# Fedomn/sqlrs

Hardware: AMD Instinct MI355X
Metric: Mrows/sec for filter->hash-join->group-by pipeline; achieved HBM GB/s vs peak (higher is better)
Workload: dtype int64 keys / f64 sum; 1 GPU; C5 filter(val>0.5) -> hash-join(fact x dim on int64 key) -> group-by(key) COUNT,SUM(f64); fact_rows=1000000000, dim_rows=10000000, groups=10000000, parallelism=single GPU

## Files before the change

sqlrs_amd/csrc/agg_partition.hip:

```cpp
#include <algorithm>
#include <cstdlib>
#include <cstring>

#include "agg_partition.hpp"
#include "device_utils.hpp"
#include "radix_part.hpp"

namespace sq {

#ifndef PART_WG_N
#define PART_WG_N 512
#endif
constexpr int PART_WG = PART_WG_N;
#ifndef DENSE_WG_N
#define DENSE_WG_N 1024
#endif
constexpr int DENSE_WG = DENSE_WG_N;
#ifndef HOT_MIN_PEERS_N
#define HOT_MIN_PEERS_N 8
#endif
constexpr int HOT_MIN_PEERS = HOT_MIN_PEERS_N;
constexpr uint64_t LDS_EMPTY = ~0ull;

__device__ __forceinline__ uint32_t bucket_of(uint64_t h, uint32_t P) {
// ... 799 lines not shown
      const int64_t st = in.nzstart[col + k];
      if (st <= lo) before++;
      else if (st < hi) {
        inside++;
        atomicOr(&gmask[(st - lo) >> 6], 1ull << ((st - lo) & 63));
      }
    }
    before = wave_sum_u32(before);
    inside = wave_sum_u32(inside);
    if (lane_id() == 0 && before) atomicAdd(&s_before, before);
    if (lane_id() == 0 && inside) atomicAdd(&s_inside, inside);
  }
  __syncthreads();
  const uint32_t k_first = s_before - 1u, k_count = s_inside + 1u;
  const bool bt_lds = !BLK && k_count <= SLIM_BT_CAP;
  const bool seg_mode = NACC == 2 && ((C0 == AK_COUNT && C1 == AK_SUM_F64) || (C0 == AK_SUM_F64 && C1 == AK_COUNT)) &&
                        hi - lo >= 4096 && (int64_t)k_count * 2048 <= hi - lo && !prm.seg_off && !BLK;
  if (bt_lds)
    for (uint32_t k = threadIdx.x; k < k_count; k += DENSE_WG) gbt[k] = in.nzbt[col + min(k_first + k, nruns - 1)];
  if (!BLK) {
    constexpr uint32_t GPT = 8;
    uint32_t carry = s_before - 1u;
    for (uint32_t g0 = 0; g0 < ngroups; g0 += DENSE_WG * GPT) {
      const uint32_t gb = g0 + threadIdx.x * GPT;
      uint32_t pc[GPT], sum = 0;
#pragma unroll
      for (uint32_t i = 0; i < GPT; i++) {
        pc[i] = gb + i < ngroups ? (uint32_t)__popcll(gmask[gb + i]) : 0u;
        sum += pc[i];
      }
      const uint32_t inc = wave_iscan_u32(sum);
      if (lane_id() == 63) s_wsum[wave_id()] = inc;
      __syncthreads();
      uint32_t wbase = 0, tot = 0;
      for (int w = 0; w < DENSE_WG / 64; w++) {
        if (w < wave_id()) wbase += s_wsum[w];
        tot += s_wsum[w];
      }
      uint32_t run = carry + wbase + inc - sum;
#pragma unroll
      for (uint32_t i = 0; i < GPT; i++) {
        if (gb + i < ngroups) gpre[gb + i] = run;
        run += pc[i];
      }
      carry += tot;
      __syncthreads();
    }
  }
#ifndef SLIM_WAVE_SPAN
#define SLIM_WAVE_SPAN 1
#endif
  constexpr int64_t SLIM_USTEP = SLIM_WAVE_SPAN ? 64 : DENSE_WG;
  const int64_t slim_toff = SLIM_WAVE_SPAN ? (int64_t)wave_id() * (LDS_U * 64) + lane_id() : (int64_t)threadIdx.x;
  auto load = [&](int64_t i0, SlimAggRows &r) {
#pragma unroll
    for (int u = 0; u < LDS_U; u++) {
      const int64_t i = min(i0 + (int64_t)u * SLIM_USTEP, hi - 1);
      slim_load_nt(in.rows, i, r.w[u], r.v[u]);
      if (BLK) {
        r.bt[u] = in.blk_bt[i >> in.log_b];
        continue;
      }
      const uint32_t g = (uint32_t)((i - lo) >> 6);
      const uint32_t k = gpre[g] + (uint32_t)__popcll(gmask[g] & le_mask);
#if defined(SLIM_DBG) && (SLIM_DBG & 16)
      r.bt[u] = k;
#else
      r.bt[u] = bt_lds ? gbt[min(k - k_first, k_count - 1)] : in.nzbt[col + min(k, nruns - 1)];
#endif
    }
  };
  uint32_t hc_slot = 0xffffffffu, hc_min = 0xffffffffu;
  uint64_t hc_acc[PART_MAX_ACC];
  auto hot_flush = [&]() {
    if (hc_slot == 0xffffffffu) return;
    if (lane_id() == 0) {
      atomicMin(&tfirst[hc_slot], hc_min);
#pragma unroll
      for (int a = 0; a < PART_MAX_ACC; a++) {
        if (a >= n_acc) break;
        unsigned long long *cell = tacc + (size_t)a * R + hc_slot;
        switch (code_of(a) & 7) {
        case AK_COUNT:
        case AK_SUM_I64: atomicAdd(cell, (unsigned long long)hc_acc[a]); break;
        case AK_SUM_F64: unsafeAtomicAdd((double *)cell, __longlong_as_double((long long)hc_acc[a])); break;
        case AK_MIN_I64:
        case AK_MIN_F64: atomicMin(cell, (unsigned long long)hc_acc[a]); break;
        default: atomicMax(cell, (unsigned long long)hc_acc[a]);
        }
      }
    }
    hc_slot = 0xffffffffu;
  };
  auto hot_take = [&](uint32_t s0, uint32_t idmin) {
    if (hc_slot != s0) {
      hot_flush();
      hc_slot = s0;
      hc_min = 0xffffffffu;
#pragma unroll
      for (int a = 0; a < PART_MAX_ACC; a++) {
        if (a >= n_acc) break;
        hc_acc[a] = acc_identity_cell(code_of(a) & 7);
      }
    }
    hc_min = idmin < hc_min ? idmin : hc_min;
  };
  auto hot_add = [&](int a, int kind, uint64_t red) {
    switch (kind) {
    case AK_COUNT:
    case AK_SUM_I64: hc_acc[a] += red; break;
    case AK_SUM_F64: hc_acc[a] = (uint64_t)__double_as_longlong(__longlong_as_double((long long)hc_acc[a]) + __longlong_as_double((long long)red)); break;
    case AK_MIN_I64:
    case AK_MIN_F64: hc_acc[a] = red < hc_acc[a] ? red : hc_acc[a]; break;
    default: hc_acc[a] = red > hc_acc[a] ? red : hc_acc[a];
    }
  };
  SlimAggRows cur, nxt;
  if (lo < hi) load(lo + slim_toff, cur);
  __builtin_amdgcn_s_waitcnt(0x0F70);
  for (int64_t base = lo; base < hi; base += (int64_t)LDS_U * DENSE_WG) {
    const int64_t i0 = base + slim_toff;
    load(i0 + (int64_t)LDS_U * DENSE_WG, nxt);
    uint32_t sl[LDS_U], id[LDS_U], tf[LDS_U];
#pragma unroll
    for (int u = 0; u < LDS_U; u++) {
      const uint32_t w = cur.w[u];
      sl[u] = w & mask;
      id[u] = (cur.bt[u] + (w >> (rbits + 13))) * in.tile + ((w >> rbits) & lmask);
      tf[u] = tfirst[sl[u]];
    }
    constexpr bool SEG_CAPABLE = NACC == 2 && ((C0 == AK_COUNT && C1 == AK_SUM_F64) || (C0 == AK_SUM_F64 && C1 == AK_COUNT));
    const int lane = (int)lane_id();
    auto seg_rows = [&](bool act, uint32_t sl_u, uint64_t v_u, uint32_t id_u, uint32_t tf_u) {
      const uint32_t key = act ? sl_u : (0x80000000u | (uint32_t)lane);
      const uint32_t prevk = (uint32_t)__builtin_amdgcn_update_dpp(0, (int)key, 0x138, 0xf, 0xf, false);
      const uint64_t bm = __ballot(lane == 0 || key != prevk);
      const int headl = 63 - __builtin_clzll(bm & le_mask);
      double incl = act ? __longlong_as_double((long long)v_u) : 0.0;
      uint32_t idh = act ? id_u : 0xffffffffu;
      wave_seg_iscan_f64_min_u32(incl, idh, headl, lane);
      const bool tail = act && (lane == 63 || ((bm >> (lane + 1)) & 1ull));
      if (tail) {
        const uint32_t s = sl_u;
        if (idh < tf_u) atomicMin(&tfirst[s], idh);
        atomicAdd(tacc + (size_t)(C0 == AK_COUNT ? 0 : 1) * R + s, (unsigned long long)(lane - headl + 1));
        unsafeAtomicAdd((double *)(tacc + (size_t)(C0 == AK_COUNT ? 1 : 0) * R + s), incl);
      }
    };
    if (seg_mode) {
#pragma unroll
      for (int u = 0; u < LDS_U; u++) {
        const bool act = i0 + (int64_t)u * SLIM_USTEP < hi;
        {
          const uint32_t s0 = (uint32_t)__builtin_amdgcn_readfirstlane((int)sl[u]);
          if (__ballot(act && sl[u] == s0) == ~0ull) {
            hot_take(s0, wave_min_u32_dpp(id[u]));
            hot_add(C0 == AK_COUNT ? 0 : 1, AK_COUNT, 64ull);
            hot_add(C0 == AK_COUNT ? 1 : 0, AK_SUM_F64, (uint64_t)__double_as_longlong(wave_sum_f64_dpp(__longlong_as_double((long long)cur.v[u]))));
            continue;
          }
        }
        seg_rows(act, sl[u], cur.v[u], id[u], tf[u]);
      }
      cur = nxt;
      continue;
    }
#pragma unroll
    for (int u = 0; u < LDS_U; u++) {
      const uint32_t s = sl[u];
      bool act = i0 + (int64_t)u * SLIM_USTEP < hi;
      if (BLK) act = act && cur.w[u] != 0xffffffffu;
#ifdef SLIM_DBG
      uint64_t actm = (SLIM_DBG & 1) ? 0ull : __ballot(act);
#else
      uint64_t actm = __ballot(act);
#endif
      for (int it = 0; it < 3 && actm; it++) {
        const int first = __builtin_ctzll(actm);
        const uint32_t s0 = (uint32_t)__builtin_amdgcn_readlane((int)s, first);
        const bool hot = act && s == s0;
        const uint64_t peers = __ballot(hot);
        if (__popcll(peers) < HOT_MIN_PEERS) break;
// ... 596 lines not shown
```

sqlrs_amd/csrc/radix_part.hip:

```cpp
#include <cstdio>
#include <cstdlib>

#include "device_utils.hpp"
#include "radix_part.hpp"
#include "radix_part_kernels.hpp"

namespace sq {

namespace {

struct Level {
  std::vector<int64_t> seg_mat, seg_start;
  std::vector<uint32_t> seg_tiles, seg_tile_base;
  int64_t mat_entries = 0;
  uint32_t num_tiles = 0, nseg = 0;
  std::vector<uint8_t> blob;
  BufP dev, tiles;
  const int64_t *d_seg_start = nullptr, *d_seg_mat = nullptr;
  const uint32_t *d_seg_tiles = nullptr, *d_seg_tile_base = nullptr;
};

Level plan_level(const std::vector<int64_t> &seg_start, uint32_t digits, int RP_TILE) {
  Level L;
  L.seg_start = seg_start;
// ... 191 lines not shown
  auto run_level = [&](int level, uint32_t digits, const std::vector<int64_t> &seg_start, const RpIn &rin,
                       const RpOut &rout, BufP *offs_out, Level *L) {
    *L = plan_level(seg_start, digits, RP_TILE);
    L->tiles = ctx->alloc(sizeof(Tile) * (size_t)std::max<uint32_t>(L->num_tiles, 1));
    upload_level(ctx, *L);
    rp_make_tiles_kernel<<<dim3((unsigned)L->seg_tiles.size()), dim3(256), 0, ctx->stream>>>(
        L->d_seg_start, L->d_seg_mat, L->d_seg_tiles, L->d_seg_tile_base, RP_TILE, (Tile *)L->tiles->p);
    SQ_HIP(hipGetLastError());
    exec_level(level, digits, *L, rin, rout, n, offs_out);
  };

  auto bucket_starts = [&](const Level &L, const BufP &offs, uint32_t digits, int64_t rows,
                           std::vector<uint32_t> *host) -> BufP {
    uint32_t nseg = L.nseg;
    int64_t total = (int64_t)nseg * digits + 1;
    BufP bs = ctx->alloc(4 * (size_t)total);
    rp_bucket_starts_kernel<<<dim3((unsigned)ceil_div(total, 256)), dim3(256), 0, ctx->stream>>>(
        offs->as<uint32_t>(), L.d_seg_mat, L.d_seg_tiles, L.d_seg_start, digits, nseg, rows, bs->as<uint32_t>());
    SQ_HIP(hipGetLastError());
    if (4 * (size_t)total <= ctx->pinned_bytes) {
      const uint32_t *h = (const uint32_t *)ctx->fetch(bs->p, 4 * (size_t)total);
      host->assign(h, h + total);
      return bs;
    }
    host->resize((size_t)total);
    SQ_HIP(hipMemcpyAsync(host->data(), bs->p, 4 * (size_t)total, hipMemcpyDeviceToHost, ctx->stream));
    ctx->sync();
    return bs;
  };

  struct EarlyStarts {
    BufP bs;
    int64_t total = 0;
    std::function<void(const BufP &)> queue;
  };
  auto early_starts_for = [&](const Level &L, uint32_t digits, int64_t rows, EarlyStarts &es) {
    es.total = (int64_t)L.nseg * digits + 1;
    const char *es_e = hook("SQLRS_RP_EARLY_STARTS");
    const bool off = es_e && es_e[0] == '0';
    es.queue = [&L, &es, digits, rows, off, ctx](const BufP &offs) {
      if (off) return;
      BufP bs = ctx->alloc(4 * (size_t)es.total);
      rp_bucket_starts_kernel<<<dim3((unsigned)ceil_div(es.total, 256)), dim3(256), 0, ctx->stream>>>(
          offs->as<uint32_t>(), L.d_seg_mat, L.d_seg_tiles, L.d_seg_start, digits, L.nseg, rows, bs->as<uint32_t>());
      SQ_HIP(hipGetLastError());
      if (ctx->fetch_early(bs->p, 4 * (size_t)es.total)) es.bs = bs;
    };
  };
  auto finish_starts = [&](EarlyStarts &es, const Level &L, const BufP &offs, uint32_t digits, int64_t rows, std::vector<uint32_t> *host) -> BufP {
    if (!es.bs) return bucket_starts(L, offs, digits, rows, host);
    const uint32_t *h = (const uint32_t *)ctx->fetch_early_wait();
    host->assign(h, h + es.total);
    return es.bs;
  };

  const char *claim_e = hook("SQLRS_RP_CLAIM");
  const int claim_env = claim_e ? std::atoi(claim_e) : -1;
  const bool claimable = p2_bits == 0 && pack && kp.dense && nv <= 1 && P <= (uint32_t)WG && P >= 2 &&
                         claim_env != 0 && (claim_env == 1 || n >= (1ll << 22));
  if (claimable) {
    const uint32_t tiles1c = (uint32_t)ceil_div(n, RP_TILE);
    uint32_t wgs = std::min<uint32_t>(tiles1c, (uint32_t)ctx->num_cus);
    if (const char *wg_e = hook("SQLRS_RP_CHUNK_WGS"))
      wgs = std::max(1u, std::min<uint32_t>(wgs, (uint32_t)std::atoi(wg_e)));
    const uint32_t tpw = (uint32_t)ceil_div(tiles1c, std::max(wgs, 1u));
    wgs = (uint32_t)ceil_div(tiles1c, std::max(tpw, 1u));
    uint32_t B = 16;
    while (B < 256 && (uint64_t)(2 * B) * 16 * wgs * P <= (uint64_t)n) B *= 2;
    const uint32_t slack = 4096 + wgs * B;
    const uint64_t slots_max = (uint64_t)n + (uint64_t)n / 8 + (uint64_t)P * ((uint64_t)slack + B) + 64;
    const uint64_t pool_rows = slots_max + (uint64_t)1024 * wgs;
    if (pool_rows <= 0xffffffffull) {
      BufP est = ctx->alloc_zero(4 * ((size_t)P + 1));
      const size_t plan_words = 3 * (size_t)P + (P & 1), plan_bytes = 4 * plan_words + 16;
      BufP plan = ctx->alloc(plan_bytes);
      SQ_HIP(hipMemsetAsync(plan->as<uint8_t>() + 4 * plan_words, 0, 16, ctx->stream));
      uint32_t *rstart = plan->as<uint32_t>(), *rend = rstart + P, *cursor = rend + P;
      uint64_t *cst = (uint64_t *)(plan->as<uint32_t>() + plan_words);
      {
        ProfScope ps(ctx, "rp_sample_hist");
        uint32_t sdiv = 8;
        while (sdiv < 32 && (int64_t)P * 4096 * (2 * sdiv) <= n) sdiv *= 2;
        const int64_t samples = (int64_t)tiles1c * (RP_TILE / sdiv);
        const unsigned sblocks = (unsigned)std::max<int64_t>(1, std::min<int64_t>(ceil_div(samples, 256 * 4 * 2), 4 * (int64_t)ctx->num_cus));
        rp_sample_hist_kernel<<<dim3(sblocks), dim3(256), 0, ctx->stream>>>(in.keys, in.filter, n, (uint32_t)RP_TILE, tiles1c, P, kp, sdiv,
                                                                           est->as<uint32_t>());
        rp_region_plan_kernel<<<dim3(1), dim3(512), 0, ctx->stream>>>(est->as<uint32_t>(), P, n, slack, B, rstart, rend, cursor);
        SQ_HIP(hipGetLastError());
      }
      const char *cslim_e = hook("SQLRS_RP_SLIM");
      const bool claim_slim = nv == 1 && kp.rbits + SLIM_LOCAL_BITS + 7 <= 32 && !(cslim_e && std::atoi(cslim_e) == 0);
      Cols cc;
      PartitionedRows::Slim csl;
      if (claim_slim) {
        uint32_t log_b = 0;
        while ((1u << log_b) < B) log_b++;
        csl.buf0 = ctx->alloc(8 * (size_t)pool_rows);
        csl.buf1 = ctx->alloc(4 * (size_t)pool_rows);
        csl.rows.v = csl.buf0->as<uint64_t>();
        csl.rows.w = csl.buf1->as<uint32_t>();
        csl.blk_bt = ctx->alloc(4 * (size_t)((slots_max >> log_b) + 2));
        csl.log_b = log_b;
        csl.tile = (uint32_t)RP_TILE;
        csl.on = true;
      } else if (use_rec) cc.rec = ctx->alloc(16 * (size_t)pool_rows);
      else {
// ... 115 lines not shown
        v.v = b0->as<uint64_t>();
        v.w = b1->as<uint32_t>();
        return v;
      };
      BufP cb0, cb1;
      BufP clen = ctx->alloc_zero(4 * (size_t)max_chunks);
      BufP cdig = ctx->alloc(4 * (size_t)max_chunks), cbase = ctx->alloc(4 * (size_t)max_chunks);
      BufP cstart = ctx->alloc(2 * (size_t)max_chunks * SLIM_RUNS);
      SQ_HIP(hipMemsetAsync(cstart->p, 0xff, 2 * (size_t)max_chunks * SLIM_RUNS, ctx->stream));
      BufP ctr = ctx->alloc_zero(8);
      BufP chist = ctx->alloc(4 * (size_t)max_chunks * digits2);
      SlimChunkOut so;
      so.rows = slim_alloc(pool_rows, cb0, cb1);
      so.chunk_len = clen->as<uint32_t>();
      so.chunk_dig = cdig->as<uint32_t>();
      so.chunk_base = cbase->as<uint32_t>();
      so.cstart = cstart->as<uint16_t>();
      so.counter = ctr->as<unsigned int>();
      so.max_chunks = (uint32_t)max_chunks;
      so.cap = (uint32_t)CAP;
      so.arena = (uint32_t)arena;
      so.hist = chist->as<uint32_t>();
      so.kshift = kp.rbits + p2_bits;
      so.max_delta = slim_delta;
      {
        const char *cc_e = hook("SQLRS_RP_CONC");
        so.conc_eighths = cc_e ? (uint32_t)std::max(1, std::min(std::atoi(cc_e), 9)) : 3u;
      }
      const int psrc = !in.filter.col ? -1 : ((const void *)in.filter.col == in.vals[0] ? 1 : 3);
      const size_t clds = (size_t)RP_TILE * 14 + (size_t)WG * (4 + 4 + 8 + 8 + 4 + 4) + (size_t)P * 4;
      {
        ProfScope ps(ctx, in.filter.col ? "rp_chunk_scatter_filter" : "rp_chunk_scatter");
        const int64_t sink = (int64_t)max_chunks * (CAP + RP_CHUNK_SKEW);
        const size_t clds768 = (size_t)RP_TILE * 14 + (size_t)768 * (4 + 4 + 8 + 8 + 4 + 4) + (size_t)P * 4;
#define SQ_SL(W, R, PS, LDS)                                                                                        \
  do {                                                                                                              \
    auto kfn = rp_chunk_scatter_slim_kernel<W, R, PS>;                                                              \
    allow_big_lds(ctx, kfn);                                                                                        \
    kfn<<<dim3(cwgs), dim3(W), LDS, ctx->stream>>>(in.keys, (const uint64_t *)in.vals[0], in.filter, n, so, P, p2_bits, d1, \
                                                   tiles1, ctpw, sink, kp);                                         \
  } while (0)
        if (psrc < 0) SQ_SL(768, 8, -1, clds768); else if (psrc == 1) SQ_SL(768, 8, 1, clds768); else SQ_SL(512, 12, 3, clds);
#undef SQ_SL
        SQ_HIP(hipGetLastError());
      }
      Level L2;
      L2.nseg = d1;
      const LevelLayout lay(d1);
      L2.dev = ctx->alloc(lay.total);
      bind_level(L2, lay);
      L2.tiles = ctx->alloc(sizeof(Tile) * (size_t)max_chunks);
      BufP totals = ctx->alloc(24);
      BufP tile_chunk = ctx->alloc(4 * (size_t)max_chunks);
      BufP plan = ctx->alloc(sizeof(ChunkPlan));
      SQ_HIP(hipMemsetAsync(plan->p, 0, sizeof(ChunkPlan), ctx->stream));
      const unsigned pblocks = (unsigned)std::min<uint64_t>(ceil_div((int64_t)max_chunks, 256 * 8), 128);
      rp_chunk_count_kernel<<<dim3(pblocks), dim3(256), 0, ctx->stream>>>(so.chunk_len, so.chunk_dig, so.counter, so.max_chunks,
                                                                        so.max_chunks, (uint32_t)RP_TILE, plan->as<ChunkPlan>());
      rp_chunk_prefix_kernel<<<dim3(1), dim3(64), 0, ctx->stream>>>(
          plan->as<ChunkPlan>(), so.counter, d1, digits2, (int64_t *)L2.d_seg_start, (int64_t *)L2.d_seg_mat,
          (uint32_t *)L2.d_seg_tiles, (uint32_t *)L2.d_seg_tile_base, totals->as<uint64_t>());
      rp_chunk_assign_kernel<<<dim3(pblocks), dim3(256), 0, ctx->stream>>>(
          so.chunk_len, so.chunk_dig, so.counter, so.max_chunks, so.max_chunks, digits2, (uint32_t)CAP, (uint32_t)RP_TILE,
          L2.d_seg_tiles, L2.d_seg_tile_base, plan->as<ChunkPlan>(), (Tile *)L2.tiles->p, tile_chunk->as<uint32_t>());
      SQ_HIP(hipGetLastError());
      const uint64_t *ht = (const uint64_t *)ctx->fetch(totals->p, 24);
      const uint64_t ntiles = ht[0], kept = ht[1], overflow = ht[2];
      if (overflow) return false;
      L2.num_tiles = (uint32_t)ntiles;
      L2.mat_entries = (int64_t)ntiles * digits2;
      out->n = (int64_t)kept;
      out->P = P;
      if (kept == 0) {
        out->bstart_host.assign((size_t)P + 1, 0u);
        out->bstart = nullptr;
        return true;
      }
      const size_t np = (size_t)kept + 1024;
      PartitionedRows::Slim &sl = out->slim;
      sl = PartitionedRows::Slim();
      sl.rows = slim_alloc(np, sl.buf0, sl.buf1);
      SlimLaunch sln;
      sln.in.rows = so.rows;
      sln.in.tile_chunk = tile_chunk->as<uint32_t>();
      sln.in.cstart = so.cstart;
      sln.out.rows = sl.rows;
      sln.kshift = so.kshift;
      sln.rbits = kp.rbits;
      BufP offs2;
      BufP premat = ctx->alloc(4 * (size_t)L2.mat_entries);
      rp_hist_from_chunks_kernel<<<dim3((unsigned)ceil_div(L2.mat_entries, 256)), dim3(256), 0, ctx->stream>>>(
          so.hist, tile_chunk->as<uint32_t>(), L2.mat_entries, digits2, premat->as<uint32_t>());
      SQ_HIP(hipGetLastError());
      EarlyStarts es;
      early_starts_for(L2, digits2, (int64_t)kept, es);
      exec_level(2, digits2, L2, RpIn(), RpOut(), (int64_t)kept, &offs2, premat, &sln, &es.queue);
      sl.nzstart = ctx->alloc(4 * (size_t)L2.mat_entries);
      sl.nzbt = ctx->alloc(4 * (size_t)L2.mat_entries);
      sl.nzcount = ctx->alloc(4 * (size_t)P);
      sl.bcol = ctx->alloc(4 * (size_t)P);
      ProfScope ps_runs(ctx, "rp_slim_runs");
      rp_slim_runs_kernel<<<dim3(P), dim3(256), 0, ctx->stream>>>(
          offs2->as<uint32_t>(), L2.mat_entries, sln.total->as<uint64_t>(), L2.d_seg_mat, L2.d_seg_tiles, L2.d_seg_tile_base,
          tile_chunk->as<uint32_t>(), so.chunk_base, digits2, sl.nzstart->as<uint32_t>(), sl.nzbt->as<uint32_t>(),
          sl.nzcount->as<uint32_t>(), sl.bcol->as<uint32_t>());
      SQ_HIP(hipGetLastError());
      if (hook("SQLRS_RP_TRACE"))
        std::fprintf(stderr, "[rp_slim] keys %p vals %p chunks %p %p rows %p %p kept %llu tiles %u\n", (const void *)in.keys, in.vals[0],
                     cb0 ? cb0->p : nullptr, cb1 ? cb1->p : nullptr, sl.buf0 ? sl.buf0->p : nullptr, sl.buf1 ? sl.buf1->p : nullptr,
                     (unsigned long long)kept, L2.num_tiles);
      sl.tile = (uint32_t)RP_TILE;
      sl.on = true;
      out->key = out->v0 = out->v1 = out->idx = out->flags = out->rec = nullptr;
      out->bstart = finish_starts(es, L2, offs2, digits2, (int64_t)kept, &out->bstart_host);
      return true;
    }
    if (chunked) {
// ... 29 lines not shown
        const uint64_t *k = in.keys, *a0 = (const uint64_t *)in.vals[0], *a1 = (const uint64_t *)in.vals[1];
        const int64_t sink = (int64_t)max_chunks * (CAP + RP_CHUNK_SKEW);
#define SQ_CS1(NV, R, PK, PS)                                                                                       \
  do {                                                                                                              \
    auto kfn = rp_chunk_scatter_kernel<NV, 512, R, PK, PS>;                                                         \
    if (NV == 1 && PK && h2) kfn = rp_chunk_scatter_kernel<NV, 512, R, PK, PS, (NV == 1 && PK)>;                    \
    allow_big_lds(ctx, kfn);                                                                                        \
    kfn<<<dim3(cwgs), dim3(512), clds, ctx->stream>>>(k, a0, a1, in.filter, n, co, P, p2_bits, d1, tiles1, ctpw,   \
                                                      sink, kp);                                                    \
  } while (0)
#define SQ_CS(NV, R, PK)                                                                                            \
  do {                                                                                                              \
    if (psrc < 0) SQ_CS1(NV, R, PK, -1);                                                                            \
    else if (psrc == 1 && NV >= 1) SQ_CS1(NV, R, PK, (NV >= 1 ? 1 : 3));                                            \
    else SQ_CS1(NV, R, PK, 3);                                                                                      \
  } while (0)
        if (nv == 2) SQ_CS(2, 8, false);
        else if (nv == 0) { if (pack) SQ_CS(0, 12, true); else SQ_CS(0, 12, false); }
        else if (!pack && h2) {
#define SQ_CH(PS)                                                                                                   \
  do {                                                                                                              \
    auto kfn = rp_chunk_scatter_kernel<1, 512, 12, false, PS, true>;                                                \
    allow_big_lds(ctx, kfn, 159 * 1024);                                                                            \
    kfn<<<dim3(cwgs), dim3(512), clds, ctx->stream>>>(k, a0, a1, in.filter, n, co, P, p2_bits, d1, tiles1, ctpw, sink, kp); \
  } while (0)
          if (psrc < 0) SQ_CH(-1); else SQ_CH(1);
#undef SQ_CH
        }
        else if (!pack && psrc != 3) {
          const size_t clds768 = (size_t)RP_TILE * (8 * (1 + nv) + 4 + 2) + (size_t)768 * (4 + 4 + 8 + 8) + (clds - ((size_t)RP_TILE * (8 * (1 + nv) + 4 + 2) + (size_t)WG * (4 + 4 + 8 + 8)));
#define SQ_CG(PS)                                                                                                   \
  do {                                                                                                              \
    auto kfn = rp_chunk_scatter_kernel<1, 768, 8, false, PS>;                                                       \
    allow_big_lds(ctx, kfn);                                                                                        \
    kfn<<<dim3(cwgs), dim3(768), clds768, ctx->stream>>>(k, a0, a1, in.filter, n, co, P, p2_bits, d1, tiles1, ctpw, sink, kp); \
  } while (0)
          if (psrc < 0) SQ_CG(-1); else if (psrc == 1) SQ_CG(1); else SQ_CG(3);
#undef SQ_CG
        }
        else if (pack) SQ_CS(1, 12, true); else SQ_CS1(1, 12, false, 3);
#undef SQ_CS
#undef SQ_CS1
        SQ_HIP(hipGetLastError());
      }
      const uint32_t digits2 = 1u << p2_bits;
      Level L2;
      L2.nseg = d1;
      const LevelLayout lay(d1);
      L2.dev = ctx->alloc(lay.total);
      bind_level(L2, lay);
      L2.tiles = ctx->alloc(sizeof(Tile) * (size_t)max_chunks);
      BufP totals = ctx->alloc(24);
      BufP tile_chunk = h2 ? ctx->alloc(4 * (size_t)max_chunks) : nullptr;
      BufP plan = ctx->alloc(sizeof(ChunkPlan));
      SQ_HIP(hipMemsetAsync(plan->p, 0, sizeof(ChunkPlan), ctx->stream));
      const unsigned pblocks = (unsigned)std::min<uint64_t>(ceil_div((int64_t)max_chunks, 256 * 8), 128);
      rp_chunk_count_kernel<<<dim3(pblocks), dim3(256), 0, ctx->stream>>>(co.chunk_len, co.chunk_dig, co.counter, co.base_chunks,
                                                                        co.max_chunks, (uint32_t)RP_TILE, plan->as<ChunkPlan>());
      rp_chunk_prefix_kernel<<<dim3(1), dim3(64), 0, ctx->stream>>>(
          plan->as<ChunkPlan>(), co.counter, d1, digits2, (int64_t *)L2.d_seg_start, (int64_t *)L2.d_seg_mat,
          (uint32_t *)L2.d_seg_tiles, (uint32_t *)L2.d_seg_tile_base, totals->as<uint64_t>());
      rp_chunk_assign_kernel<<<dim3(pblocks), dim3(256), 0, ctx->stream>>>(
          co.chunk_len, co.chunk_dig, co.counter, co.base_chunks, co.max_chunks, digits2, (uint32_t)CAP, (uint32_t)RP_TILE,
          L2.d_seg_tiles, L2.d_seg_tile_base, plan->as<ChunkPlan>(), (Tile *)L2.tiles->p,
          tile_chunk ? tile_chunk->as<uint32_t>() : nullptr);
      SQ_HIP(hipGetLastError());
      const uint64_t *ht = (const uint64_t *)ctx->fetch(totals->p, 24);
      const uint64_t ntiles = ht[0], kept = ht[1], overflow = ht[2];
      if (overflow) return false;
      L2.num_tiles = (uint32_t)ntiles;
      L2.mat_entries = (int64_t)ntiles * digits2;
      out->n = (int64_t)kept;
      out->P = P;
      RpIn rin2;
      rin2.key = ck->as<uint64_t>();
      rin2.v0 = co.v0;
      rin2.v1 = co.v1;
      rin2.idx = co.idx;
      rin2.flags = nullptr;
      rin2.key_validity = rin2.v0_validity = rin2.v1_validity = nullptr;
      Cols c2;
      RpOut rout2;
      alloc_cols((int64_t)kept, true, c2, rout2);
      BufP offs2, premat;
      if (h2 && L2.mat_entries) {
        premat = ctx->alloc(4 * (size_t)L2.mat_entries);
        rp_hist_from_chunks_kernel<<<dim3((unsigned)ceil_div(L2.mat_entries, 256)), dim3(256), 0, ctx->stream>>>(
            co.hist, tile_chunk->as<uint32_t>(), L2.mat_entries, digits2, premat->as<uint32_t>());
        SQ_HIP(hipGetLastError());
      }
      EarlyStarts es;
      early_starts_for(L2, digits2, (int64_t)kept, es);
      exec_level(2, digits2, L2, rin2, rout2, (int64_t)kept, &offs2, premat, nullptr, &es.queue);
      publish(c2);
      out->bstart = finish_starts(es, L2, offs2, digits2, (int64_t)kept, &out->bstart_host);
      return true;
    }
  }

  Cols c1;
  RpOut rout;
  alloc_cols(n, p2_bits == 0, c1, rout);
  RpIn rin;
  rin.key = in.keys;
  rin.v0 = (const uint64_t *)in.vals[0];
  rin.v1 = (const uint64_t *)in.vals[1];
  rin.idx = nullptr;
  rin.flags = nullptr;
  rin.key_validity = in.key_validity;
  rin.v0_validity = in.val_validity[0];
  rin.v1_validity = in.val_validity[1];
  BufP offs1;
  Level L1;
  run_level(1, d1, {0, n}, rin, rout, &offs1, &L1);
  std::vector<uint32_t> hs;
  BufP bs1 = bucket_starts(L1, offs1, d1, n, &hs);
  out->n = n;
  out->P = P;
// ... 27 lines not shown
```

sqlrs_amd/csrc/radix_part_kernels.hpp:

```cpp
#pragma once
#include "device_utils.hpp"
#include "radix_part.hpp"

#ifdef RP_NT_STORES
#define RP_ST(ptr, val) __builtin_nontemporal_store((val), (ptr))
#else
#define RP_ST(ptr, val) (*(ptr) = (val))
#endif

namespace sq {


constexpr int vmcnt_imm(int n) { return (n & 0xF) | ((n >> 4) << 14) | 0x0F70; }

struct Tile {
  int64_t start;
  uint32_t len;
  uint32_t stride;
  int64_t mat;
};

__device__ __forceinline__ uint32_t xcd_tile(uint32_t b, uint32_t nb) {
  uint32_t q = nb >> 3, r = nb & 7, x = b & 7, i = b >> 3;
  return x * q + min(x, r) + i;
// ... 1335 lines not shown
    const uint32_t d = min((uint32_t)sdig[p], (uint32_t)(RP_WG - 1));
    int64_t g = (p < split[d] ? gb0[d] : gb1[d]) + p;
    if (p >= len || g < 0) g = sink + (int64_t)blockIdx.x * RP_WG + threadIdx.x;
    slim_store(out.rows, g, sw[p], sv0[p]);
  };

  if (t0 < t1) {
    uint32_t len = tile_len(t0);
    cur_tile = t0;
    rp_chunk_load<1, RP_WG, RP_ROWS, PSRC>(key, v0, nullptr, flt.col, tile_start(t0), len, nxt);
    __builtin_amdgcn_s_waitcnt(0x0F70);
    take_rows(len, t0, true, cur);
    cnt[threadIdx.x] = 0;
    __syncthreads();
#pragma unroll
    for (int j = 0; j < RP_ROWS; j++) rank_row(j);
    __syncthreads();
    scan_and_stage();
    uint32_t staged_len = s_total;
    uint32_t tcur = min(t0 + 1, t1 - 1);
    len = tile_len(tcur);
    cur_tile = tcur;
    rp_chunk_load<1, RP_WG, RP_ROWS, PSRC>(key, v0, nullptr, flt.col, tile_start(tcur), len, nxt);
    __builtin_amdgcn_s_waitcnt(0x0F70);
    take_rows(len, tcur, tcur != t0, cur);
    for (uint32_t ti = t0 + 1; ti < t1; ti++) {
      const uint32_t tnext = min(ti + 1, t1 - 1);
      const uint32_t nlen = tile_len(tnext);
      rp_chunk_load<1, RP_WG, RP_ROWS, PSRC>(key, v0, nullptr, flt.col, tile_start(tnext), nlen, nxt);
      cnt[threadIdx.x] = 0;
      __syncthreads();
#pragma unroll
      for (int j = 0; j < RP_ROWS; j++) {
        if ((uint32_t)(j * RP_WG) < staged_len) store_row(j, staged_len);
        rank_row(j);
      }
      __builtin_amdgcn_s_waitcnt(0x0F70);
      __syncthreads();
      scan_and_stage();
      staged_len = s_total;
      take_rows(nlen, tnext, tnext != ti, cur);
      cur_tile = tnext;
    }
#pragma unroll
    for (int j = 0; j < RP_ROWS; j++)
      if ((uint32_t)(j * RP_WG) < staged_len) store_row(j, staged_len);
  }
  if (owner && !dead) fill_sentinels(pos, room);
  if (threadIdx.x == 0 && kept) atomicAdd(out.kept, kept);
}

struct ChunkPlan {
  uint32_t seg_tiles[512];
  uint32_t cursor[512];
  unsigned long long seg_rows[512];
};
__global__ __launch_bounds__(256) void rp_chunk_count_kernel(const uint32_t *__restrict__ chunk_len,
                                                             const uint32_t *__restrict__ chunk_dig,
                                                             const unsigned int *__restrict__ counter, uint32_t base_chunks,
                                                             uint32_t max_chunks, uint32_t tile, ChunkPlan *plan) {
  __shared__ uint32_t s_tiles[512];
  __shared__ unsigned long long s_rows[512];
  for (uint32_t i = threadIdx.x; i < 512; i += 256) {
    s_tiles[i] = 0;
    s_rows[i] = 0;
  }
  __syncthreads();
  const uint32_t nchunks = min(base_chunks + counter[0], max_chunks);
  for (uint32_t c = blockIdx.x * 256 + threadIdx.x; c < nchunks; c += gridDim.x * 256) {
    const uint32_t len = chunk_len[c];
    if (!len) continue;
    atomicAdd(&s_tiles[chunk_dig[c]], (len + tile - 1) / tile);
    atomicAdd(&s_rows[chunk_dig[c]], (unsigned long long)len);
  }
  __syncthreads();
  for (uint32_t i = threadIdx.x; i < 512; i += 256) {
    if (s_tiles[i]) atomicAdd(&plan->seg_tiles[i], s_tiles[i]);
    if (s_rows[i]) atomicAdd(&plan->seg_rows[i], s_rows[i]);
  }
}
__global__ __launch_bounds__(64) void rp_chunk_prefix_kernel(const ChunkPlan *plan, const unsigned int *__restrict__ counter,
                                                             uint32_t nseg, uint32_t digits2, int64_t *__restrict__ seg_start,
                                                             int64_t *__restrict__ seg_mat, uint32_t *__restrict__ seg_tiles,
                                                             uint32_t *__restrict__ seg_tile_base,
                                                             uint64_t *__restrict__ totals ) {
  if (threadIdx.x != 0) return;
  uint32_t tb = 0;
  int64_t rows = 0;
  for (uint32_t s = 0; s < nseg; s++) {
    seg_start[s] = rows;
    seg_tile_base[s] = tb;
    seg_mat[s] = (int64_t)tb * digits2;
    seg_tiles[s] = plan->seg_tiles[s];
    tb += plan->seg_tiles[s];
    rows += (int64_t)plan->seg_rows[s];
  }
  seg_start[nseg] = rows;
  totals[0] = tb;
  totals[1] = (uint64_t)rows;
  totals[2] = counter[1];
}
__global__ __launch_bounds__(256) void rp_chunk_assign_kernel(const uint32_t *__restrict__ chunk_len,
                                                              const uint32_t *__restrict__ chunk_dig,
                                                              const unsigned int *__restrict__ counter, uint32_t base_chunks,
                                                              uint32_t max_chunks, uint32_t digits2, uint32_t cap, uint32_t tile,
                                                              const uint32_t *__restrict__ seg_tiles,
                                                              const uint32_t *__restrict__ seg_tile_base, ChunkPlan *plan,
                                                              Tile *__restrict__ tiles, uint32_t *__restrict__ tile_chunk) {
  __shared__ uint32_t s_need[512], s_base[512];
  const uint32_t nchunks = min(base_chunks + counter[0], max_chunks);
  for (uint32_t c0 = blockIdx.x * 256; c0 < nchunks; c0 += gridDim.x * 256) {
    for (uint32_t i = threadIdx.x; i < 512; i += 256) s_need[i] = 0;
    __syncthreads();
    const uint32_t c = c0 + threadIdx.x;
    const uint32_t len = c < nchunks ? chunk_len[c] : 0;
    const uint32_t s = len ? chunk_dig[c] : 0, nt = (len + tile - 1) / tile;
    const uint32_t local = len ? atomicAdd(&s_need[s], nt) : 0;
    __syncthreads();
    for (uint32_t i = threadIdx.x; i < 512; i += 256)
      if (s_need[i]) s_base[i] = atomicAdd(&plan->cursor[i], s_need[i]);
    __syncthreads();
    if (len) {
      const uint32_t base = seg_tile_base[s], i0 = s_base[s] + local;
      for (uint32_t q = 0; q < nt; q++) {
        Tile t;
        t.start = (int64_t)c * (cap + RP_CHUNK_SKEW) + (int64_t)q * tile;
        t.len = min(tile, len - q * tile);
        t.stride = seg_tiles[s];
        t.mat = (int64_t)base * digits2 + i0 + q;
        tiles[base + i0 + q] = t;
        if (tile_chunk) tile_chunk[base + i0 + q] = c;
      }
    }
    __syncthreads();
  }
}
__global__ void rp_hist_from_chunks_kernel(const uint32_t *__restrict__ hist, const uint32_t *__restrict__ tile_chunk,
                                           int64_t entries, uint32_t digits, uint32_t *__restrict__ mat) {
  const int64_t i = blockIdx.x * (int64_t)blockDim.x + threadIdx.x;
  if (i >= entries) return;
  const uint32_t t = (uint32_t)(i / digits), d = (uint32_t)(i % digits);
  mat[i] = hist[(size_t)tile_chunk[t] * digits + d];
}

__global__ void rp_bucket_starts_kernel(const uint32_t *__restrict__ offs,
                                        const int64_t *__restrict__ seg_mat,
                                        const uint32_t *__restrict__ seg_tiles,
                                        const int64_t *__restrict__ seg_start, uint32_t digits,
                                        uint32_t nseg, int64_t n, uint32_t *__restrict__ bstart) {
  int64_t b = blockIdx.x * (int64_t)blockDim.x + threadIdx.x;
  int64_t total = (int64_t)nseg * digits;
  if (b > total) return;
  if (b == total) {
    bstart[b] = (uint32_t)n;
    return;
  }
  uint32_t s = (uint32_t)(b / digits), d = (uint32_t)(b % digits);
  bstart[b] = seg_tiles[s] ? offs[seg_mat[s] + (int64_t)d * seg_tiles[s]] : (uint32_t)seg_start[s + 1];
}

__global__ void rp_make_tiles_kernel(const int64_t *__restrict__ seg_start, const int64_t *__restrict__ seg_mat,
                                     const uint32_t *__restrict__ seg_tiles, const uint32_t *__restrict__ seg_tile_base,
                                     int rp_tile, Tile *__restrict__ tiles) {
  const uint32_t s = blockIdx.x, nt = seg_tiles[s], base = seg_tile_base[s];
  const int64_t start = seg_start[s], end = seg_start[s + 1], mat = seg_mat[s];
  for (uint32_t i = threadIdx.x; i < nt; i += blockDim.x) {
    Tile t;
    t.start = start + (int64_t)i * rp_tile;
    t.len = (uint32_t)min((int64_t)rp_tile, end - t.start);
    t.stride = nt;
    t.mat = mat + i;
    tiles[base + i] = t;
  }
}

}
```

Baseline: 92770 Mrows/s.

## Make chunk tile planning deterministic via per-block scans; defer base-tile lookup in slim agg

Chunk-to-tile planning is rebuilt. A per-block count kernel now writes per-segment partial counts, a per-segment prefix kernel scans them, and an assign kernel computes segment bases and writes tiles using wave-level ranking. This replaces the global atomics, the memset and the single-thread serial prefix kernel. Separately, the slim aggregation kernel loads one base tile per wave and computes per-row ids only when a row's first-seen slot could be beaten, which skips most popcount and LDS lookups. The trade-offs are extra scratch allocations, one assign grid block per 256 chunks, and 32-bit row counts per segment.

```diff
diff --git a/sqlrs_amd/csrc/agg_partition.hip b/sqlrs_amd/csrc/agg_partition.hip
--- a/sqlrs_amd/csrc/agg_partition.hip
+++ b/sqlrs_amd/csrc/agg_partition.hip
@@ -875,23 +875,20 @@
 #endif
   constexpr int64_t SLIM_USTEP = SLIM_WAVE_SPAN ? 64 : DENSE_WG;
   const int64_t slim_toff = SLIM_WAVE_SPAN ? (int64_t)wave_id() * (LDS_U * 64) + lane_id() : (int64_t)threadIdx.x;
+  auto base_tile_at = [&](int64_t i) {
+    const uint32_t g = (uint32_t)((i - lo) >> 6);
+    const uint32_t k = gpre[g] + (uint32_t)__popcll(gmask[g] & ((2ull << ((i - lo) & 63)) - 1ull));
+    return bt_lds ? gbt[min(k - k_first, k_count - 1)] : in.nzbt[col + min(k, nruns - 1)];
+  };
   auto load = [&](int64_t i0, SlimAggRows &r) {
 #pragma unroll
     for (int u = 0; u < LDS_U; u++) {
       const int64_t i = min(i0 + (int64_t)u * SLIM_USTEP, hi - 1);
       slim_load_nt(in.rows, i, r.w[u], r.v[u]);
-      if (BLK) {
+      if (BLK)
         r.bt[u] = in.blk_bt[i >> in.log_b];
-        continue;
-      }
-      const uint32_t g = (uint32_t)((i - lo) >> 6);
-      const uint32_t k = gpre[g] + (uint32_t)__popcll(gmask[g] & le_mask);
-#if defined(SLIM_DBG) && (SLIM_DBG & 16)
-      r.bt[u] = k;
-#else
-      r.bt[u] = bt_lds ? gbt[min(k - k_first, k_count - 1)] : in.nzbt[col + min(k, nruns - 1)];
-#endif
-    }
+    }
+    if (!BLK) r.bt[0] = base_tile_at(min(i0 - (int64_t)lane_id(), hi - 1));
   };
   uint32_t hc_slot = 0xffffffffu, hc_min = 0xffffffffu;
   uint64_t hc_acc[PART_MAX_ACC];
@@ -949,8 +946,26 @@
     for (int u = 0; u < LDS_U; u++) {
       const uint32_t w = cur.w[u];
       sl[u] = w & mask;
-      id[u] = (cur.bt[u] + (w >> (rbits + 13))) * in.tile + ((w >> rbits) & lmask);
       tf[u] = tfirst[sl[u]];
+      if (BLK) id[u] = (cur.bt[u] + (w >> (rbits + 13))) * in.tile + ((w >> rbits) & lmask);
+    }
+    if (!BLK) {
+      const uint32_t bound = cur.bt[0] * in.tile;
+      bool late = false;
+#pragma unroll
+      for (int u = 0; u < LDS_U; u++) {
+        id[u] = 0xffffffffu;
+        late = late || tf[u] >= bound;
+      }
+      if (__ballot(late)) {
+#pragma unroll
+        for (int u = 0; u < LDS_U; u++) {
+          if (tf[u] < bound) continue;
+          const uint32_t w = cur.w[u];
+          const uint32_t bt = base_tile_at(min(i0 + (int64_t)u * SLIM_USTEP, hi - 1));
+          id[u] = (bt + (w >> (rbits + 13))) * in.tile + ((w >> rbits) & lmask);
+        }
+      }
     }
     constexpr bool SEG_CAPABLE = NACC == 2 && ((C0 == AK_COUNT && C1 == AK_SUM_F64) || (C0 == AK_SUM_F64 && C1 == AK_COUNT));
     const int lane = (int)lane_id();
diff --git a/sqlrs_amd/csrc/radix_part.hip b/sqlrs_amd/csrc/radix_part.hip
--- a/sqlrs_amd/csrc/radix_part.hip
+++ b/sqlrs_amd/csrc/radix_part.hip
@@ -267,6 +267,24 @@
     const uint32_t *h = (const uint32_t *)ctx->fetch_early_wait();
     host->assign(h, h + es.total);
     return es.bs;
+  };
+  std::vector<BufP> plan_scratch;
+  auto plan_chunk_tiles = [&](const uint32_t *chunk_len, const uint32_t *chunk_dig, const unsigned int *counter, uint32_t base_chunks,
+                              uint32_t max_chunks, uint32_t digits2, uint32_t cap, uint32_t nseg, const Level &L2, uint64_t *totals,
+                              uint32_t *tile_chunk) {
+    const unsigned nb = (unsigned)ceil_div((int64_t)max_chunks, 256);
+    BufP blk_tiles = ctx->alloc(4 * (size_t)nb * nseg), blk_rows = ctx->alloc(4 * (size_t)nb * nseg);
+    BufP plan = ctx->alloc(sizeof(ChunkPlan));
+    plan_scratch.insert(plan_scratch.end(), {blk_tiles, blk_rows, plan});
+    rp_chunk_count_kernel<<<dim3(nb), dim3(256), 0, ctx->stream>>>(chunk_len, chunk_dig, counter, base_chunks, max_chunks,
+                                                                 (uint32_t)RP_TILE, nseg, blk_tiles->as<uint32_t>(),
+                                                                 blk_rows->as<uint32_t>());
+    rp_chunk_prefix_kernel<<<dim3(nseg), dim3(64), 0, ctx->stream>>>(nb, blk_tiles->as<uint32_t>(), blk_rows->as<uint32_t>(),
+                                                                   plan->as<ChunkPlan>());
+    rp_chunk_assign_kernel<<<dim3(nb), dim3(256), 0, ctx->stream>>>(
+        chunk_len, chunk_dig, counter, base_chunks, max_chunks, digits2, cap, (uint32_t)RP_TILE, nseg, blk_tiles->as<uint32_t>(),
+        plan->as<ChunkPlan>(), (int64_t *)L2.d_seg_start, (int64_t *)L2.d_seg_mat, (uint32_t *)L2.d_seg_tiles,
+        (uint32_t *)L2.d_seg_tile_base, totals, (Tile *)L2.tiles->p, tile_chunk);
   };
 
   const char *claim_e = hook("SQLRS_RP_CLAIM");
@@ -488,17 +506,8 @@
       L2.tiles = ctx->alloc(sizeof(Tile) * (size_t)max_chunks);
       BufP totals = ctx->alloc(24);
       BufP tile_chunk = ctx->alloc(4 * (size_t)max_chunks);
-      BufP plan = ctx->alloc(sizeof(ChunkPlan));
-      SQ_HIP(hipMemsetAsync(plan->p, 0, sizeof(ChunkPlan), ctx->stream));
-      const unsigned pblocks = (unsigned)std::min<uint64_t>(ceil_div((int64_t)max_chunks, 256 * 8), 128);
-      rp_chunk_count_kernel<<<dim3(pblocks), dim3(256), 0, ctx->stream>>>(so.chunk_len, so.chunk_dig, so.counter, so.max_chunks,
-                                                                        so.max_chunks, (uint32_t)RP_TILE, plan->as<ChunkPlan>());
-      rp_chunk_prefix_kernel<<<dim3(1), dim3(64), 0, ctx->stream>>>(
-          plan->as<ChunkPlan>(), so.counter, d1, digits2, (int64_t *)L2.d_seg_start, (int64_t *)L2.d_seg_mat,
-          (uint32_t *)L2.d_seg_tiles, (uint32_t *)L2.d_seg_tile_base, totals->as<uint64_t>());
-      rp_chunk_assign_kernel<<<dim3(pblocks), dim3(256), 0, ctx->stream>>>(
-          so.chunk_len, so.chunk_dig, so.counter, so.max_chunks, so.max_chunks, digits2, (uint32_t)CAP, (uint32_t)RP_TILE,
-          L2.d_seg_tiles, L2.d_seg_tile_base, plan->as<ChunkPlan>(), (Tile *)L2.tiles->p, tile_chunk->as<uint32_t>());
+      plan_chunk_tiles(so.chunk_len, so.chunk_dig, so.counter, so.max_chunks, so.max_chunks, digits2, (uint32_t)CAP, d1, L2,
+                       totals->as<uint64_t>(), tile_chunk->as<uint32_t>());
       SQ_HIP(hipGetLastError());
       const uint64_t *ht = (const uint64_t *)ctx->fetch(totals->p, 24);
       const uint64_t ntiles = ht[0], kept = ht[1], overflow = ht[2];
@@ -634,18 +643,8 @@
       L2.tiles = ctx->alloc(sizeof(Tile) * (size_t)max_chunks);
       BufP totals = ctx->alloc(24);
       BufP tile_chunk = h2 ? ctx->alloc(4 * (size_t)max_chunks) : nullptr;
-      BufP plan = ctx->alloc(sizeof(ChunkPlan));
-      SQ_HIP(hipMemsetAsync(plan->p, 0, sizeof(ChunkPlan), ctx->stream));
-      const unsigned pblocks = (unsigned)std::min<uint64_t>(ceil_div((int64_t)max_chunks, 256 * 8), 128);
-      rp_chunk_count_kernel<<<dim3(pblocks), dim3(256), 0, ctx->stream>>>(co.chunk_len, co.chunk_dig, co.counter, co.base_chunks,
-                                                                        co.max_chunks, (uint32_t)RP_TILE, plan->as<ChunkPlan>());
-      rp_chunk_prefix_kernel<<<dim3(1), dim3(64), 0, ctx->stream>>>(
-          plan->as<ChunkPlan>(), co.counter, d1, digits2, (int64_t *)L2.d_seg_start, (int64_t *)L2.d_seg_mat,
-          (uint32_t *)L2.d_seg_tiles, (uint32_t *)L2.d_seg_tile_base, totals->as<uint64_t>());
-      rp_chunk_assign_kernel<<<dim3(pblocks), dim3(256), 0, ctx->stream>>>(
-          co.chunk_len, co.chunk_dig, co.counter, co.base_chunks, co.max_chunks, digits2, (uint32_t)CAP, (uint32_t)RP_TILE,
-          L2.d_seg_tiles, L2.d_seg_tile_base, plan->as<ChunkPlan>(), (Tile *)L2.tiles->p,
-          tile_chunk ? tile_chunk->as<uint32_t>() : nullptr);
+      plan_chunk_tiles(co.chunk_len, co.chunk_dig, co.counter, co.base_chunks, co.max_chunks, digits2, (uint32_t)CAP, d1, L2,
+                       totals->as<uint64_t>(), tile_chunk ? tile_chunk->as<uint32_t>() : nullptr);
       SQ_HIP(hipGetLastError());
       const uint64_t *ht = (const uint64_t *)ctx->fetch(totals->p, 24);
       const uint64_t ntiles = ht[0], kept = ht[1], overflow = ht[2];
diff --git a/sqlrs_amd/csrc/radix_part_kernels.hpp b/sqlrs_amd/csrc/radix_part_kernels.hpp
--- a/sqlrs_amd/csrc/radix_part_kernels.hpp
+++ b/sqlrs_amd/csrc/radix_part_kernels.hpp
@@ -1411,87 +1411,142 @@
 
 struct ChunkPlan {
   uint32_t seg_tiles[512];
-  uint32_t cursor[512];
-  unsigned long long seg_rows[512];
+  uint32_t seg_rows[512];
 };
 __global__ __launch_bounds__(256) void rp_chunk_count_kernel(const uint32_t *__restrict__ chunk_len,
                                                              const uint32_t *__restrict__ chunk_dig,
                                                              const unsigned int *__restrict__ counter, uint32_t base_chunks,
-                                                             uint32_t max_chunks, uint32_t tile, ChunkPlan *plan) {
-  __shared__ uint32_t s_tiles[512];
-  __shared__ unsigned long long s_rows[512];
+                                                             uint32_t max_chunks, uint32_t tile, uint32_t nseg,
+                                                             uint32_t *__restrict__ blk_tiles, uint32_t *__restrict__ blk_rows) {
+  __shared__ uint32_t s_tiles[512], s_rows[512];
   for (uint32_t i = threadIdx.x; i < 512; i += 256) {
     s_tiles[i] = 0;
     s_rows[i] = 0;
   }
   __syncthreads();
   const uint32_t nchunks = min(base_chunks + counter[0], max_chunks);
-  for (uint32_t c = blockIdx.x * 256 + threadIdx.x; c < nchunks; c += gridDim.x * 256) {
-    const uint32_t len = chunk_len[c];
-    if (!len) continue;
-    atomicAdd(&s_tiles[chunk_dig[c]], (len + tile - 1) / tile);
-    atomicAdd(&s_rows[chunk_dig[c]], (unsigned long long)len);
+  const uint32_t c = blockIdx.x * 256 + threadIdx.x;
+  const uint32_t len = c < nchunks ? chunk_len[c] : 0;
+  if (len) {
+    const uint32_t s = min(chunk_dig[c], 511u);
+    atomicAdd(&s_tiles[s], (len + tile - 1) / tile);
+    atomicAdd(&s_rows[s], len);
   }
   __syncthreads();
-  for (uint32_t i = threadIdx.x; i < 512; i += 256) {
-    if (s_tiles[i]) atomicAdd(&plan->seg_tiles[i], s_tiles[i]);
-    if (s_rows[i]) atomicAdd(&plan->seg_rows[i], s_rows[i]);
-  }
-}
-__global__ __launch_bounds__(64) void rp_chunk_prefix_kernel(const ChunkPlan *plan, const unsigned int *__restrict__ counter,
-                                                             uint32_t nseg, uint32_t digits2, int64_t *__restrict__ seg_start,
-                                                             int64_t *__restrict__ seg_mat, uint32_t *__restrict__ seg_tiles,
-                                                             uint32_t *__restrict__ seg_tile_base,
-                                                             uint64_t *__restrict__ totals ) {
-  if (threadIdx.x != 0) return;
-  uint32_t tb = 0;
-  int64_t rows = 0;
-  for (uint32_t s = 0; s < nseg; s++) {
-    seg_start[s] = rows;
-    seg_tile_base[s] = tb;
-    seg_mat[s] = (int64_t)tb * digits2;
-    seg_tiles[s] = plan->seg_tiles[s];
-    tb += plan->seg_tiles[s];
-    rows += (int64_t)plan->seg_rows[s];
-  }
-  seg_start[nseg] = rows;
-  totals[0] = tb;
-  totals[1] = (uint64_t)rows;
-  totals[2] = counter[1];
+  for (uint32_t i = threadIdx.x; i < nseg; i += 256) {
+    blk_tiles[(size_t)i * gridDim.x + blockIdx.x] = s_tiles[i];
+    blk_rows[(size_t)i * gridDim.x + blockIdx.x] = s_rows[i];
+  }
+}
+__global__ __launch_bounds__(64) void rp_chunk_prefix_kernel(uint32_t nb, uint32_t *__restrict__ blk_tiles,
+                                                             const uint32_t *__restrict__ blk_rows, ChunkPlan *plan) {
+  uint32_t *bt = blk_tiles + (size_t)blockIdx.x * nb;
+  const uint32_t *br = blk_rows + (size_t)blockIdx.x * nb;
+  uint32_t carry = 0, rows = 0;
+  for (uint32_t j0 = 0; j0 < nb; j0 += 64) {
+    const uint32_t j = j0 + threadIdx.x;
+    const uint32_t t = j < nb ? bt[j] : 0u;
+    rows += j < nb ? br[j] : 0u;
+    const uint32_t inc = wave_iscan_u32(t);
+    if (j < nb) bt[j] = carry + inc - t;
+    carry += (uint32_t)__builtin_amdgcn_readlane((int)inc, 63);
+  }
+  rows = wave_sum_u32(rows);
+  if (threadIdx.x == 0) {
+    plan->seg_tiles[blockIdx.x] = carry;
+    plan->seg_rows[blockIdx.x] = rows;
+  }
 }
 __global__ __launch_bounds__(256) void rp_chunk_assign_kernel(const uint32_t *__restrict__ chunk_len,
                                                               const uint32_t *__restrict__ chunk_dig,
                                                               const unsigned int *__restrict__ counter, uint32_t base_chunks,
                                                               uint32_t max_chunks, uint32_t digits2, uint32_t cap, uint32_t tile,
-                                                              const uint32_t *__restrict__ seg_tiles,
-                                                              const uint32_t *__restrict__ seg_tile_base, ChunkPlan *plan,
+                                                              uint32_t nseg, const uint32_t *__restrict__ blk_tiles,
+                                                              const ChunkPlan *__restrict__ plan,
+                                                              int64_t *__restrict__ seg_start, int64_t *__restrict__ seg_mat,
+                                                              uint32_t *__restrict__ seg_tiles, uint32_t *__restrict__ seg_tile_base,
+                                                              uint64_t *__restrict__ totals ,
                                                               Tile *__restrict__ tiles, uint32_t *__restrict__ tile_chunk) {
-  __shared__ uint32_t s_need[512], s_base[512];
+  __shared__ uint32_t s_tb[512];
+  __shared__ uint32_t s_wcnt[4][512];
+  __shared__ uint32_t s_wt[4], s_wr[4];
+  for (uint32_t i = threadIdx.x; i < 4 * 512; i += 256) (&s_wcnt[0][0])[i] = 0;
+  const uint32_t e0 = 2 * threadIdx.x, e1 = e0 + 1;
+  const uint32_t ta = e0 < nseg ? plan->seg_tiles[e0] : 0u, tb = e1 < nseg ? plan->seg_tiles[e1] : 0u;
+  const uint32_t ra = e0 < nseg ? plan->seg_rows[e0] : 0u, rb = e1 < nseg ? plan->seg_rows[e1] : 0u;
+  const uint32_t tinc = wave_iscan_u32(ta + tb), rinc = wave_iscan_u32(ra + rb);
+  if (lane_id() == 63) {
+    s_wt[wave_id()] = tinc;
+    s_wr[wave_id()] = rinc;
+  }
+  __syncthreads();
+  uint32_t tex = tinc - (ta + tb), rex = rinc - (ra + rb), ttot = 0, rtot = 0;
+  for (int w = 0; w < 4; w++) {
+    if (w < wave_id()) {
+      tex += s_wt[w];
+      rex += s_wr[w];
+    }
+    ttot += s_wt[w];
+    rtot += s_wr[w];
+  }
+  s_tb[e0] = tex;
+  s_tb[e1] = tex + ta;
+  if (blockIdx.x == 0) {
+    if (e0 < nseg) {
+      seg_start[e0] = (int64_t)rex;
+      seg_tile_base[e0] = tex;
+      seg_mat[e0] = (int64_t)tex * digits2;
+      seg_tiles[e0] = ta;
+    }
+    if (e1 < nseg) {
+      seg_start[e1] = (int64_t)rex + ra;
+      seg_tile_base[e1] = tex + ta;
+      seg_mat[e1] = (int64_t)(tex + ta) * digits2;
+      seg_tiles[e1] = tb;
+    }
+    if (threadIdx.x == 0) {
+      seg_start[nseg] = (int64_t)rtot;
+      totals[0] = ttot;
+      totals[1] = rtot;
+      totals[2] = counter[1];
+    }
+  }
   const uint32_t nchunks = min(base_chunks + counter[0], max_chunks);
-  for (uint32_t c0 = blockIdx.x * 256; c0 < nchunks; c0 += gridDim.x * 256) {
-    for (uint32_t i = threadIdx.x; i < 512; i += 256) s_need[i] = 0;
-    __syncthreads();
-    const uint32_t c = c0 + threadIdx.x;
-    const uint32_t len = c < nchunks ? chunk_len[c] : 0;
-    const uint32_t s = len ? chunk_dig[c] : 0, nt = (len + tile - 1) / tile;
-    const uint32_t local = len ? atomicAdd(&s_need[s], nt) : 0;
-    __syncthreads();
-    for (uint32_t i = threadIdx.x; i < 512; i += 256)
-      if (s_need[i]) s_base[i] = atomicAdd(&plan->cursor[i], s_need[i]);
-    __syncthreads();
-    if (len) {
-      const uint32_t base = seg_tile_base[s], i0 = s_base[s] + local;
-      for (uint32_t q = 0; q < nt; q++) {
-        Tile t;
-        t.start = (int64_t)c * (cap + RP_CHUNK_SKEW) + (int64_t)q * tile;
-        t.len = min(tile, len - q * tile);
-        t.stride = seg_tiles[s];
-        t.mat = (int64_t)base * digits2 + i0 + q;
-        tiles[base + i0 + q] = t;
-        if (tile_chunk) tile_chunk[base + i0 + q] = c;
-      }
-    }
-    __syncthreads();
+  const uint32_t c = blockIdx.x * 256 + threadIdx.x;
+  const uint32_t len = c < nchunks ? chunk_len[c] : 0;
+  const uint32_t s = len ? min(chunk_dig[c], 511u) : 0u, nt = (len + tile - 1) / tile;
+  uint32_t local = 0;
+  for (uint64_t todo = __ballot(len != 0); todo;) {
+    const int lead = __builtin_ctzll(todo);
+    const uint32_t d = (uint32_t)__builtin_amdgcn_readlane((int)s, lead);
+    const bool mine = len != 0 && s == d;
+    const uint64_t m = __ballot(mine);
+    uint32_t cnt;
+    if (__ballot(mine && nt != 1) == 0) {
+      cnt = (uint32_t)__popcll(m);
+      if (mine) local = (uint32_t)mbcnt(m);
+    } else {
+      const uint32_t v = mine ? nt : 0u, inc = wave_iscan_u32(v);
+      cnt = (uint32_t)__builtin_amdgcn_readlane((int)inc, 63);
+      if (mine) local = inc - v;
+    }
+    if (lane_id() == lead) s_wcnt[wave_id()][d] = cnt;
+    todo &= ~m;
+  }
+  __syncthreads();
+  if (len) {
+    uint32_t i0 = blk_tiles[(size_t)s * gridDim.x + blockIdx.x] + local;
+    for (int w = 0; w < wave_id(); w++) i0 += s_wcnt[w][s];
+    const uint32_t base = s_tb[s], stride = plan->seg_tiles[s];
+    for (uint32_t q = 0; q < nt; q++) {
+      Tile t;
+      t.start = (int64_t)c * (cap + RP_CHUNK_SKEW) + (int64_t)q * tile;
+      t.len = min(tile, len - q * tile);
+      t.stride = stride;
+      t.mat = (int64_t)base * digits2 + i0 + q;
+      tiles[base + i0 + q] = t;
+      if (tile_chunk) tile_chunk[base + i0 + q] = c;
+    }
   }
 }
 __global__ void rp_hist_from_chunks_kernel(const uint32_t *__restrict__ hist, const uint32_t *__restrict__ tile_chunk,
```

New measurement: 93180 Mrows/s, median of 2. No clear change (+0.4%).
